# agiresearch/OpenP5

Measured on AMD Instinct MI355X. Metric: train_samples_per_sec, higher is better.
Workload: dtype bf16; 1 GPU; ML-1M-shaped sequential prompts, t5-small V=32100, B=64/GPU L=128 T=8, dropout 0.1, fwd+bwd+clip+AdamW (BASELINE.json configs[1]); global_batch=64, seq_len=128, tgt_len=8, parallelism=dp1

## Files before the change

### include/p5hip.h

```cpp
#ifndef P5HIP_H
#define P5HIP_H
#include <stddef.h>
#include <stdint.h>

#ifdef __cplusplus
extern "C" {
#endif

typedef struct P5Config {
  int vocab_size, d_model, d_kv, d_ff, n_enc_layers, n_dec_layers, n_heads;
  int rel_buckets, rel_max_distance, whole_word_size;
  int gated_gelu;
  int dtype;
  float eps, dropout;
  int pad_id, eos_id;
} P5Config;

typedef struct P5Engine P5Engine;

const char* p5_last_error(void);
int p5_set_option(const char* name, int value);
int p5_abi_version(void);
int p5_profile_begin(void);
int p5_profile_end(char* report, int cap);
// ... 233 lines not shown
                       const int* child_col, const uint32_t* excluded, int excl_words, float temperature, int rows, int T, int ldl, int ld_ref,
                       void* stream);
int p5_op_trie_reg_bwd(int dtype, void* dlogits, const float* logits, const float* ref_logits, const float* lse, const float* entropy, const float* kl,
                       const float* lse_ref, const int64_t* labels, const int* node, const int* state, const float* dnll, const float* d_entropy,
                       const float* d_kl, const int* child_off, const int* child_tok, const int* child_node, const int* child_col,
                       const uint32_t* excluded, int excl_words, float temperature, int rows, int T, int ldl, int ld_ref, int ldd,
                       const int64_t* out_attn, float gscale, float entropy_coef, float kl_coef, void* stream);
int p5_op_trunc_ce_fwd_cols(int dtype, float* nll, float* lse, float* row_cut, int* state, const float* logits, const int64_t* labels, const int* node,
                            const int* child_off, const int* child_tok, const int* child_node, const int* child_col, const uint32_t* excluded,
                            int excl_words, float temperature, int top_k, float top_p, int rows, int T, int ldl, void* stream);
int p5_op_trunc_ce_bwd_cols(int dtype, void* dlogits, const float* logits, const float* lse, const float* row_cut, const int64_t* labels, const int* node,
                            const int* state, const float* dnll, const int* child_off, const int* child_tok, const int* child_node, const int* child_col,
                            const uint32_t* excluded, int excl_words, float temperature, int rows, int T, int ldl, int ldd, const int64_t* out_attn,
                            float gscale, void* stream);
int p5_op_masked_mean(float* loss, const float* nll, const int64_t* out_attn, int B, int T, void* stream);
int p5_policy_batch(const int64_t* sequences, const int64_t* labels, const int64_t* output_attention, const float* rewards, int B, int S, int Ts,
                    int Tg, int baseline, float policy_coef, float sft_coef, int token_sum, float adv_eps, int with_gold, int pad_id, int eos_id,
                    int64_t* labels_out, int64_t* attention_out, float* rewards_out, float* advantages, float* weights_out, float* user_stats,
                    float* stats, void* stream);
int p5_op_skinny_gemm(int dtype, int amode, const void* A, int lda, const float* ln, const void* W, int ldw, void* C, int ldc,
                      int M, int N, int K, int epi, float alpha, float eps, void* stream);
int p5_op_dec_cross_attn(int dtype, int variant, void* out, const void* q, const void* kv, const int64_t* mask, int B, int H, int Kb,
                         int L, void* stream);
int p5_op_dec_cross_attn_ex(int dtype, int variant, void* out, const void* q, const float* x, const float* ln, const void* Wq, const void* kv,
                            int ldkv, const int64_t* mask, int B, int H, int Kb, int L, int d, float eps, const int* done, void* stream);
int p5_op_dec_self_attn(int dtype, void* out, const void* qkv, void* cache, const int* anc_odd, const int* anc_even, const float* rel_table,
                        const int* lut, int lut_half, int R, int H, const int* step, int max_len, const int* done, void* stream);
int p5_op_rmsnorm_f32in(int dtype, void* y, const float* x, const float* w, int rows, int d, float eps, const int* done, void* stream);
int p5_op_head_lse(int dtype, int nv, float* part_m, float* part_s, const void* hn, const void* E, int R, int d, int V, float alpha,
                   const int* done, void* stream);
// ... 41 lines not shown
```

### openp5_amd/_abi.py

```python
import ctypes as C

c_i64p = C.POINTER(C.c_int64)
vp, i32, i64, f32, f64, u32 = C.c_void_p, C.c_int, C.c_int64, C.c_float, C.c_double, C.c_uint32


class P5Config(C.Structure):
    _fields_ = [
        ("vocab_size", i32), ("d_model", i32), ("d_kv", i32), ("d_ff", i32), ("n_enc_layers", i32),
        ("n_dec_layers", i32), ("n_heads", i32), ("rel_buckets", i32), ("rel_max_distance", i32),
        ("whole_word_size", i32), ("gated_gelu", i32), ("dtype", i32), ("eps", f32), ("dropout", f32),
        ("pad_id", i32), ("eos_id", i32),
    ]


class P5GemmProblem(C.Structure):
    _fields_ = [("A", vp), ("B", vp), ("C", vp), ("aux", vp), ("M", i32), ("N", i32), ("K", i32), ("lda", i32), ("ldb", i32), ("ldc", i32),
                ("ldaux", i32), ("epi", i32), ("c_f32", i32), ("splitk", i32), ("alpha", f32), ("rowss", vp), ("rowss_eps", f32), ("ssq_out", vp), ("rowss_nt", i32), ("ssq_nt", i32),
                ("C2", vp), ("ldc2", i32), ("gate_F", i32),
                ("nb_dot", vp), ("nb_dot_nt", i32), ("nb_rin", vp), ("nb_rout", vp), ("nb_w", vp), ("nb_dw", vp)]


class P5EmbedBwdSet(C.Structure):
    _fields_ = [("key0", vp), ("key1", vp), ("dres0", vp), ("dres1", vp), ("n0", i32), ("n1", i32), ("site0", u32), ("site1", u32),
                ("drop_p0", f32), ("drop_p1", f32), ("table", vp), ("idx", vp), ("csort", vp), ("part", vp)]
# ... 101 lines not shown
    "p5_op_trie_ce_fwd": (i32, [i32, vp, vp, vp, vp, vp, vp, vp, vp, vp, vp, i32, f32, i32, i32, i32, vp]),
    "p5_op_trie_ce_bwd": (i32, [i32, vp, vp, vp, vp, vp, vp, vp, vp, vp, vp, vp, i32, f32, i32, i32, i32, i32, vp, f32, vp]),
    "p5_op_trunc_cut": (i32, [vp, vp, vp, vp, vp, vp, vp, vp, i32, f32, i32, f32, i32, i32, i32, vp]),
    "p5_op_trunc_ce_fwd": (i32, [i32, vp, vp, vp, vp, vp, vp, vp, vp, vp, vp, vp, i32, f32, i32, f32, i32, i32, i32, vp]),
    "p5_op_trunc_ce_bwd": (i32, [i32, vp, vp, vp, vp, vp, vp, vp, vp, vp, vp, vp, vp, i32, f32, i32, i32, i32, i32, vp, f32, vp]),
    "p5_op_item_gather": (i32, [i32, vp, vp, vp, i32, i32, vp]),
    "p5_op_item_scatter": (i32, [vp, vp, vp, i32, i32, i32, i32, vp]),
    "p5_op_trie_ce_fwd_cols": (i32, [i32, vp, vp, vp, vp, vp, vp, vp, vp, vp, vp, vp, i32, f32, i32, i32, i32, vp]),
    "p5_op_trie_ce_bwd_cols": (i32, [i32, vp, vp, vp, vp, vp, vp, vp, vp, vp, vp, vp, vp, i32, f32, i32, i32, i32, i32, vp, f32, vp]),
    "p5_op_trie_reg_fwd": (i32, [i32, vp, vp, vp, vp, vp, vp, vp, vp, vp, vp, vp, vp, vp, vp, vp, i32, f32, i32, i32, i32, i32, vp]),
    "p5_op_trie_reg_bwd": (i32, [i32, vp, vp, vp, vp, vp, vp, vp, vp, vp, vp, vp, vp, vp, vp, vp, vp, vp, vp, i32, f32, i32, i32, i32, i32, i32, vp, f32,
                                 f32, f32, vp]),
    "p5_op_trunc_ce_fwd_cols": (i32, [i32, vp, vp, vp, vp, vp, vp, vp, vp, vp, vp, vp, vp, i32, f32, i32, f32, i32, i32, i32, vp]),
    "p5_op_trunc_ce_bwd_cols": (i32, [i32, vp, vp, vp, vp, vp, vp, vp, vp, vp, vp, vp, vp, vp, i32, f32, i32, i32, i32, i32, vp, f32, vp]),
    "p5_op_masked_mean": (i32, [vp, vp, vp, i32, i32, vp]),
    "p5_policy_batch": (i32, [vp, vp, vp, vp, i32, i32, i32, i32, i32, f32, f32, i32, f32, i32, i32, i32, vp, vp, vp, vp, vp, vp, vp, vp]),
    "p5_op_dec_cross_attn": (i32, [i32, i32, vp, vp, vp, vp, i32, i32, i32, i32, vp]),
    "p5_op_skinny_gemm": (i32, [i32, i32, vp, i32, vp, vp, i32, vp, i32, i32, i32, i32, i32, f32, f32, vp]),
    "p5_op_dec_cross_attn_ex": (i32, [i32, i32, vp, vp, vp, vp, vp, vp, i32, vp, i32, i32, i32, i32, i32, f32, vp, vp]),
    "p5_op_dec_self_attn": (i32, [i32, vp, vp, vp, vp, vp, vp, vp, i32, i32, i32, vp, i32, vp, vp]),
    "p5_op_rmsnorm_f32in": (i32, [i32, vp, vp, vp, i32, i32, f32, vp, vp]),
    "p5_op_head_lse": (i32, [i32, i32, vp, vp, vp, vp, i32, i32, i32, f32, vp, vp]),
    "p5_op_dec_score": (i32, [i32, i32, vp, vp, i32, vp, vp, i32, f32, vp, i32, i32, vp, vp, vp, vp, vp, vp, i32, i32, i32, i32, i32, vp, vp, vp, vp, vp, vp]),
    "p5_op_head_nv": (i32, [i32, i32]),
    "p5_op_rank_select": (i32, [i32, vp, vp, i64, vp, i32, i32, vp, vp, i32, i32, vp, vp, vp, vp]),
    "p5_op_rank_edges": (i32, [i32, i32, vp, i64, vp, vp, i32, i32, vp, i32, vp, i32, i32, i32, i32, vp, vp, i32, vp, vp, vp]),
    "p5_op_cand_row_lse": (i32, [i32, i32, vp, vp, vp, i32, i32, vp, i32, i32, vp]),
    "p5_op_tree_attn": (i32, [i32, i32, vp, vp, vp, vp, i32, i32, i32, i32, i32, vp, vp, i32, vp, vp, i32, i32, vp]),
    "p5_op_cand_plan": (i32, [vp, vp, vp, vp, vp, vp, i32, i32, i32, i32, i32, i32, vp]),
    "p5_op_cand_rows": (i32, [vp, vp, i32, i32, i32, vp, vp, i32, i32, vp]),
# ... 30 lines not shown
```

### openp5_amd/csrc/p5_elem.h

```cpp
#pragma once
#include "p5_device.h"
#include "p5_rng.h"

template <class T>
__global__ __launch_bounds__(256) void p5_embed_fwd_kernel(T* __restrict__ out, const T* __restrict__ E, const T* __restrict__ WW,
                                                          const int64_t* __restrict__ ids, const int64_t* __restrict__ ww,
                                                          int rows, int d, P5Drop drop, float* __restrict__ ssq_part = nullptr) {
  constexpr int EPF = TT<T>::EPF;
  const int lane = threadIdx.x & 63;
  const int row = blockIdx.x * 4 + (threadIdx.x >> 6);
  if (row >= rows) return;
  const int64_t id = ids[row];
  const int64_t w = WW ? ww[row] : 0;
  const bool do_drop = drop.state != nullptr && drop.thr != 0;
  const uint32_t seed = p5_seed(drop);
  for (int c = lane; c < d / EPF; c += 64) {
    float x[8], y[8];
    unpack16<T>(ld16(E + (size_t)id * d + c * EPF), x);
    if (WW) {
      unpack16<T>(ld16(WW + (size_t)w * d + c * EPF), y);
#pragma unroll
      for (int e = 0; e < EPF; ++e) x[e] += y[e];
    }
    if (do_drop) {
#pragma unroll
      for (int e = 0; e < EPF; ++e)
        x[e] = p5_keep(seed, drop.site_key, (uint32_t)(row * d + c * EPF + e), drop.thr) ? x[e] * drop.scale : 0.f;
// ... 533 lines not shown
```

### openp5_amd/csrc/p5_embed.h

```cpp
#pragma once
#include "p5_device.h"
#include "p5_rng.h"

typedef int i32x4 __attribute__((ext_vector_type(4)));
#define P5_EMB_SEG 32
#define P5_EMB_MAXSETS 2

struct P5EmbSet {
  const int64_t* key0; const int64_t* key1;
  const float* dres0; const float* dres1;
  P5Drop drop0, drop1;
  float* table;
  int n0, n1;
  int* perm; int* sstart; int* slen;
  int* skey;
  unsigned long long* csort;
  float* part;
};
struct P5EmbArgs {
  P5EmbSet s[P5_EMB_MAXSETS];
  int nsets, d;
};

__device__ static __forceinline__ int emb_key(const P5EmbSet& s, int r) { return (int)(r < s.n0 ? s.key0[r] : s.key1[r - s.n0]); }
// ... 9 lines not shown
  __syncthreads();
  for (int k = 2; k <= P5_EMB_CHUNK; k <<= 1) {
    for (int j = k >> 1; j > 0; j >>= 1) {
      const int i = threadIdx.x, l = i ^ j;
      if (l > i) {
        const unsigned long long x = sv[i], y = sv[l];
        const bool up = (i & k) == 0;
        if ((x > y) == up) { sv[i] = y; sv[l] = x; }
      }
      __syncthreads();
    }
  }
  s.csort[(size_t)blockIdx.x * P5_EMB_CHUNK + threadIdx.x] = sv[threadIdx.x];
}

__device__ static __forceinline__ int emb_lower_bound(const unsigned long long* v, int m, unsigned long long x) {
  int lo = 0, hi = m;
#pragma unroll 1
  while (lo < hi) {
    const int mid = (lo + hi) >> 1;
    if (v[mid] < x) lo = mid + 1; else hi = mid;
  }
  return lo;
}

__global__ __launch_bounds__(256) void p5_embed_rank_kernel(P5EmbArgs a) {
  constexpr int CPB = 16;
  __shared__ unsigned long long sc[CPB * P5_EMB_CHUNK];
  __shared__ int scnt[3][4][64];
  const P5EmbSet& s = a.s[blockIdx.y];
  const int n = s.n0 + s.n1;
  if (blockIdx.x * 64 >= n) return;
  const int lane = threadIdx.x & 63, wave = threadIdx.x >> 6;
  const int r = blockIdx.x * 64 + lane;
  const int k = r < n ? emb_key(s, r) : 0;
  const unsigned long long me = (((unsigned long long)(unsigned)k) << 32) | (unsigned)r;
  const unsigned long long klo = ((unsigned long long)(unsigned)k) << 32, khi = ((unsigned long long)(unsigned)k + 1ull) << 32;
  const int nchunks = (n + P5_EMB_CHUNK - 1) / P5_EMB_CHUNK;
  int pos = 0, start = 0, end = 0;
  for (int c0 = 0; c0 < nchunks; c0 += CPB) {
    const int nc = nchunks - c0 < CPB ? nchunks - c0 : CPB;
    __syncthreads();
    for (int i = threadIdx.x; i < nc * P5_EMB_CHUNK; i += 256) sc[i] = s.csort[(size_t)c0 * P5_EMB_CHUNK + i];
    __syncthreads();
    for (int c = wave; c < nc; c += 4) {
      const unsigned long long* v = sc + c * P5_EMB_CHUNK;
      const int lo = emb_lower_bound(v, P5_EMB_CHUNK, klo);
      start += lo;
      const int hi = lo + emb_lower_bound(v + lo, P5_EMB_CHUNK - lo, khi);
      end += hi;
      pos += lo + emb_lower_bound(v + lo, hi - lo, me);
    }
  }
  scnt[0][wave][lane] = pos; scnt[1][wave][lane] = start; scnt[2][wave][lane] = end;
  __syncthreads();
  if (wave == 0 && r < n) {
    pos = scnt[0][0][lane] + scnt[0][1][lane] + scnt[0][2][lane] + scnt[0][3][lane];
    start = scnt[1][0][lane] + scnt[1][1][lane] + scnt[1][2][lane] + scnt[1][3][lane];
    end = scnt[2][0][lane] + scnt[2][1][lane] + scnt[2][2][lane] + scnt[2][3][lane];
    s.perm[pos] = r; s.skey[pos] = k; s.sstart[pos] = start; s.slen[pos] = end - start;
  }
}

__device__ static __forceinline__ void emb_row2(const P5EmbSet& s, int r, int d, int c, uint32_t seed0, uint32_t seed1, float& x0, float& x1) {
  const bool first = r < s.n0;
  const int lr = first ? r : r - s.n0;
  const float* src = (first ? s.dres0 : s.dres1) + (size_t)lr * d + c;
  const P5Drop& dp = first ? s.drop0 : s.drop1;
  x0 = src[0]; x1 = src[1];
  if (dp.state != nullptr && dp.thr != 0) {
    const uint32_t seed = first ? seed0 : seed1;
    const uint32_t i0 = (uint32_t)(lr * d + c);
    x0 = p5_keep(seed, dp.site_key, i0, dp.thr) ? x0 * dp.scale : 0.f;
    x1 = p5_keep(seed, dp.site_key, i0 + 1, dp.thr) ? x1 * dp.scale : 0.f;
  }
}

__global__ __launch_bounds__(256) void p5_embed_seg_kernel(P5EmbArgs a) {
  constexpr int S = P5_EMB_SEG;
  __shared__ int sp[S], sk[S], sst[S], sln[S];
  const P5EmbSet& s = a.s[blockIdx.y];
  const int n = s.n0 + s.n1, d = a.d;
  const int p0 = blockIdx.x * S;
  if (p0 >= n) return;
  const int cnt = n - p0 < S ? n - p0 : S;
  if (threadIdx.x < S) {
    const int p = p0 + threadIdx.x;
    const bool ok = threadIdx.x < cnt;
    sp[threadIdx.x] = ok ? s.perm[p] : 0; sk[threadIdx.x] = ok ? s.skey[p] : -1;
    sst[threadIdx.x] = ok ? s.sstart[p] : 0; sln[threadIdx.x] = ok ? s.slen[p] : 0;
  }
  __syncthreads();
  const uint32_t seed0 = p5_seed(s.drop0), seed1 = p5_seed(s.drop1);
  for (int c = threadIdx.x * 2; c < d; c += 512) {
    float v0[S], v1[S];
#pragma unroll
    for (int j = 0; j < S; ++j) {
      v0[j] = 0.f; v1[j] = 0.f;
      if (j < cnt) emb_row2(s, sp[j], d, c, seed0, seed1, v0[j], v1[j]);
    }
    float o0[S], o1[S];
#pragma unroll
    for (int j = 0; j < S; ++j) {
      o0[j] = 0.f; o1[j] = 0.f;
      if (j < cnt && (j == cnt - 1 || sk[j + 1] != sk[j])) {
        const int ss = sst[j], se = ss + sln[j];
        if (ss >= p0 && se <= p0 + S) {
          const float* src = s.table + (size_t)sk[j] * d + c;
          o0[j] = src[0]; o1[j] = src[1];
        }
      }
    }
    float a0 = 0.f, a1 = 0.f;
#pragma unroll
    for (int j = 0; j < S; ++j) {
      if (j >= cnt) break;
      a0 += v0[j]; a1 += v1[j];
      const bool last = j == cnt - 1 || sk[j + 1] != sk[j];
      if (last) {
        const int ss = sst[j], se = ss + sln[j];
        const bool head = ss < p0, tail = se > p0 + S;
        float* dst = (!head && !tail) ? s.table + (size_t)sk[j] * d + c : s.part + ((size_t)blockIdx.x * 2 + (head ? 0 : 1)) * d + c;
        if (!head && !tail) { dst[0] = o0[j] + a0; dst[1] = o1[j] + a1; } else { dst[0] = a0; dst[1] = a1; }
        a0 = 0.f; a1 = 0.f;
      }
    }
  }
}

__global__ __launch_bounds__(256) void p5_embed_fix_kernel(P5EmbArgs a) {
  constexpr int S = P5_EMB_SEG;
  const P5EmbSet& s = a.s[blockIdx.y];
  const int n = s.n0 + s.n1, d = a.d;
  const int p0 = blockIdx.x * S;
  if (p0 + S >= n) return;
  const int last = p0 + S - 1;
  const int ss = s.sstart[last], se = ss + s.slen[last];
  if (se <= p0 + S || ss < p0) return;
  const int key = s.skey[last];
  const int b1 = (se - 1) / S;
  for (int c = threadIdx.x * 2; c < d; c += 512) {
// ... 18 lines not shown
```

### openp5_amd/csrc/p5_lib.hip

```cpp
#include <string>
#include <vector>
#include <cstring>
#include <cstdio>
#include <cmath>
#include <cstdlib>
#ifndef P5_EMU
#include <dlfcn.h>
#endif

#include "p5_host.h"
#include "p5_elem.h"
#include "p5_embed.h"
#include "p5_decode.h"
#include "p5_decode2.h"
#include "p5_decode_wide.h"
#include "p5_verify.h"
#include "p5_rank.h"
#include "p5_cand.h"
#include "p5_prune.h"
#include "p5_bound.h"
#include "p5_sample.h"
#include "p5_sbs.h"
#include "p5_trie_ce.h"
#include "p5_trie_reg.h"
// ... 3 lines not shown
#include "../../include/p5hip.h"

thread_local std::string g_p5_err;

static int g_opt_wgrad_group = getenv("P5_WGRAD_GROUP") ? atoi(getenv("P5_WGRAD_GROUP")) : 1;
static int g_opt_dec_nb = getenv("P5_DEC_NB") ? atoi(getenv("P5_DEC_NB")) : 0;
static int g_opt_dec_kw = getenv("P5_DEC_KW") ? atoi(getenv("P5_DEC_KW")) : 0;
static int g_opt_dec_fuseq = getenv("P5_DEC_FUSEQ") ? atoi(getenv("P5_DEC_FUSEQ")) : 1;
static int g_opt_dgrad_t = getenv("P5_DGRAD_T") ? atoi(getenv("P5_DGRAD_T")) : 1;
static int g_opt_dec_cross = getenv("P5_DEC_CROSS") ? atoi(getenv("P5_DEC_CROSS")) : 3;
static int g_opt_dec_head = getenv("P5_DEC_HEAD") ? atoi(getenv("P5_DEC_HEAD")) : 1;
static int g_opt_dec_atomic = getenv("P5_DEC_ATOMIC") ? atoi(getenv("P5_DEC_ATOMIC")) : 0;
static int g_opt_adam_tiles = getenv("P5_ADAM_TILES") ? atoi(getenv("P5_ADAM_TILES")) : 1;
static int g_opt_gen_ff = getenv("P5_GEN_FF") ? atoi(getenv("P5_GEN_FF")) : 1;
static int g_opt_dec_head_nv = getenv("P5_DEC_HEAD_NV") ? atoi(getenv("P5_DEC_HEAD_NV")) : 0;
static int g_opt_gen_wide = getenv("P5_GEN_WIDE") ? atoi(getenv("P5_GEN_WIDE")) : 0;

__global__ __launch_bounds__(256) void p5_shift_right_kernel(int64_t* out, const int64_t* labels, int B, int T, int64_t start) {
  const int i = blockIdx.x * 256 + threadIdx.x;
  if (i >= B * T) return;
  const int t = i % T;
  int64_t v = (t == 0) ? start : labels[i - 1];
  if (v == -100) v = start;
  out[i] = v;
}

__global__ __launch_bounds__(64) void p5_tr_probe_kernel(unsigned short* out, const unsigned short* in) {
  __shared__ __attribute__((aligned(16))) unsigned short lds[256];
  const int l = threadIdx.x;
  for (int i = l; i < 256; i += 64) lds[i] = in[i];
  __syncthreads();
  const u32x2 r = lds_tr16_b64(&lds[(l >> 4) * 64 + (l & 15) * 4]);
  out[l * 4 + 0] = (unsigned short)(r[0] & 0xFFFF);
  out[l * 4 + 1] = (unsigned short)(r[0] >> 16);
  out[l * 4 + 2] = (unsigned short)(r[1] & 0xFFFF);
  out[l * 4 + 3] = (unsigned short)(r[1] >> 16);
}

static constexpr int P5_MAX_STAGED = 160;
// ... 54 lines not shown
  std::vector<LayerOff> enc, dec;
  std::vector<ParamInfo> table;
  float* P = nullptr; float* G = nullptr; void* S = nullptr;
  const int* lut_enc = nullptr; const int* lut_dec = nullptr; int lut_half = 0;
  uint32_t* rng = nullptr;
  int B = 0, L = 0, T = 0, training = 0, M = 0, Md = 0, Vp = 0;
  int Gt = 1, Bd = 0;
  const float* tgt_w = nullptr;
  const int64_t *ids = nullptr, *ww = nullptr, *mask = nullptr, *labels = nullptr, *out_attn = nullptr;
  std::vector<LayerSave> es, ds;
  void *enc_x0 = nullptr, *enc_xf = nullptr, *enc_out = nullptr; float* enc_rstd_f = nullptr;
  int64_t* dec_ids = nullptr; void *dec_x0 = nullptr, *dec_xf = nullptr, *dec_hn = nullptr; float* dec_rstd_f = nullptr;
  float *logits = nullptr, *lse_tok = nullptr, *ssq_scratch = nullptr;
  float *ce_part = nullptr, *ce_lab = nullptr, *ce_g = nullptr;
  bool ce_free_fwd = false;
  struct ItemLoss {
    bool on = false; P5TrieCe tr = {nullptr, nullptr, nullptr, nullptr, 0, 1.f}; int* state_out = nullptr;
    bool trunc = false; P5TruncCe tc = {0, 1.f}; float* row_cut = nullptr;
    bool head = false; const int* head_tok = nullptr; int Nu = 0, Nup = 0;
    void* head_ws = nullptr; size_t head_ws_bytes = 0;
    void *EU = nullptr, *dlogitsU = nullptr; float *logitsU = nullptr, *dEU = nullptr;
    bool reg = false; const float* ref = nullptr; int ld_ref = 0; float* row_terms = nullptr; float ent_coef = 0.f, kl_coef = 0.f;
    float* terms_out = nullptr;
  };
  ItemLoss il_next, il;
  const float *bw_dH = nullptr, *bw_dKL = nullptr;
  void* Sf = nullptr;
  float *dres_a = nullptr, *dres_b = nullptr, *d_enc = nullptr, *Dvec = nullptr, *dres_cur = nullptr, *rel_partial = nullptr;
  void *dy = nullptr, *dn = nullptr, *dqkv = nullptr, *dO = nullptr, *dh = nullptr, *du = nullptr, *dlogits = nullptr, *dkv = nullptr;
  void *dy2[P5_NSETS] = {}, *dh2[P5_NSETS] = {}, *du2[P5_NSETS] = {}, *dqkv2[P5_NSETS] = {}, *dkv2[P5_NSETS] = {};
// ... 781 lines not shown
  const int nd_ = c.n_dec_layers, ldkv = nd_ * 2 * in;
  {
    hipStream_t ks = e->side ? e->side : s;
    if (e->side) fork_to_side(e, s);
    P5_TRY(linear_fwd<T>(ks, e->enc_out, d, Wc<T>(e, e->dec[0].ca.k), e->ds[0].kv_ca, ldkv, M, 2 * in, d));
#ifndef P5_EMU
    if (e->side) hipEventRecord(e->kv_ev[0], e->side);
#endif
    if (nd_ > 1) {
      P5_TRY(linear_fwd<T>(ks, e->enc_out, d, Wc<T>(e, e->dec[1].ca.k), e->ds[1].kv_ca, ldkv, M, (nd_ - 1) * 2 * in, d));
#ifndef P5_EMU
      if (e->side) hipEventRecord(e->kv_ev[1], e->side);
#endif
    }
  }
  P5_LAUNCH(p5_shift_right_kernel, dim3((Md + 255) / 256), dim3(256), 0, s, e->dec_ids, e->labels, e->Bd, e->T, (int64_t)c.pad_id);
  P5_TRY(P5_KCHECK());
  const bool nf = norm_fused<T>(e);
  P5_LAUNCH((p5_embed_fwd_kernel<T>), dim3((Md + 3) / 4), dim3(256), 0, s, (T*)e->dec_x0, Wc<T>(e, e->off_E), (const T*)nullptr,
            (const int64_t*)e->dec_ids, (const int64_t*)nullptr, Md, d, mk_drop(e, 1, 0, 0), nf ? e->ds[0].ssq_sa : (float*)nullptr);
  P5_TRY(P5_KCHECK());
  for (int i = 0; i < c.n_dec_layers; ++i) {
    const LayerOff& lo = e->dec[i];
    LayerSave& l = e->ds[i];
    void* xnext = (i + 1 < c.n_dec_layers) ? e->ds[i + 1].x_sa : e->dec_xf;
    float* ssq_next = (i + 1 < c.n_dec_layers) ? e->ds[i + 1].ssq_sa : e->ssq_scratch;
    if (nf) {
      P5_TRY(gemm_nf<T>(s, l.x_sa, d, Wnf<T>(e, lo.sa.q), d, l.qkv, 3 * in, Md, 3 * in, d, P5_EPI_STORE, nullptr, 0, no_drop(), l.ssq_sa, c.eps, nullptr, d));
    } else {
      P5_TRY(rmsnorm_fwd<T>(s, l.n_sa, l.rstd_sa, l.x_sa, e->P + lo.sa.ln, Md, d, c.eps, no_drop()));
      P5_TRY(linear_fwd<T>(s, l.n_sa, d, Wc<T>(e, lo.sa.q), l.qkv, 3 * in, Md, 3 * in, d));
    }
    P5AttnArgs a;
    memset(&a, 0, sizeof(a));
    a.Q = l.qkv; a.K = (const T*)l.qkv + in; a.V = (const T*)l.qkv + 2 * in; a.O = l.o_sa; a.lse = l.lse_sa;
// ... 262 lines not shown
    if (e->tr_pending && e->tr_ev) { hipStreamWaitEvent(s, e->tr_ev, 0); hipStreamWaitEvent(e->side ? e->side : s, e->tr_ev, 0); }
#endif
    e->tr_pending = false;
#ifndef P5_EMU
    if (e->zg_pending && e->zg_ev) { hipStreamWaitEvent(s, e->zg_ev, 0); if (e->side) hipStreamWaitEvent(e->side, e->zg_ev, 0); }
#endif
    e->zg_pending = false;
    if (!dnll) P5_REQUIRE(e->out_attn, "backward without dnll needs p5_forward_loss (output_attention mask)");
    struct ItemGradsOnce { P5Engine* e; ~ItemGradsOnce() { e->bw_dH = e->bw_dKL = nullptr; } } item_grads_once{e};
    const float alpha = 1.0f / sqrtf((float)d);
    const bool hd = e->il.on && e->il.head;
    const float* hd_lg = hd ? (const float*)e->il.logitsU : (const float*)e->logits;
    void* hd_dl = hd ? e->il.dlogitsU : e->dlogits;
    const int hd_ld = hd ? e->il.Nup : e->Vp;
    if (e->ce_free_fwd) {
      P5_LAUNCH(p5_ce_gscale_kernel, dim3((Md + 255) / 256), dim3(256), 0, s, e->ce_g, e->labels, dnll, e->out_attn, e->T, 1.0f / (float)e->Bd, Md, e->tgt_w);
      P5_TRY(P5_KCHECK());
      P5GemmArgs g;
      memset(&g, 0, sizeof(g));
      g.A = e->dec_hn; g.B = Wc<T>(e, e->off_E); g.C = e->dlogits; g.M = Md; g.N = c.vocab_size; g.K = d; g.lda = d; g.ldb = d; g.ldc = e->Vp;
      g.epi = P5_EPI_CE_GRAD; g.alpha = alpha; g.drop = no_drop();
      g.ce_labels = e->labels; g.ce_lse = e->lse_tok; g.ce_g = e->ce_g; g.ce_np = (c.vocab_size + 63) / 64;
      P5_TRY(launch_gemm<T>(g, s));
    } else if (e->il.on && e->il.trunc) {
      P5_LAUNCH((p5_trunc_ce_bwd_kernel<T>), dim3(Md), dim3(256), 0, s, (T*)hd_dl, hd_lg, (const float*)e->lse_tok,
                (const float*)e->il.row_cut, e->labels, (const int*)e->ce_lab, (const int*)e->ce_g, dnll, e->il.tr, hd_ld, hd_ld, e->out_attn, e->T,
                1.0f / (float)e->Bd);
      P5_TRY(P5_KCHECK());
    } else if (e->il.on && e->il.reg) {
      const float* rt = e->il.row_terms;
      P5_LAUNCH((p5_trie_reg_bwd_kernel<T>), dim3(Md), dim3(256), 0, s, (T*)hd_dl, hd_lg, e->il.ref, (const float*)e->lse_tok, rt, rt + Md,
                rt + 2 * (size_t)Md, e->labels, (const int*)e->ce_lab, (const int*)e->ce_g, dnll, e->bw_dH, e->bw_dKL, e->il.tr, hd_ld, e->il.ld_ref,
// ... 1780 lines not shown
  else if (!strcmp(name, "gemm_ws")) g_opt_gemm_ws = value;
  else if (!strcmp(name, "gemm_ws128")) g_opt_gemm_ws128 = value;
  else if (!strcmp(name, "gemm_rect")) g_opt_gemm_rect = value;
  else if (!strcmp(name, "gemm_ws128_min_k")) g_opt_gemm_ws128_min_k = value;
  else if (!strcmp(name, "gate_fuse")) g_opt_gate_fuse = value;
  else if (!strcmp(name, "norm_bwd_blocks")) g_opt_norm_bwd_blocks = value;
  else if (!strcmp(name, "norm_bwd_fuse")) g_opt_norm_bwd_fuse = value;
  else if (!strcmp(name, "adam_tiles")) g_opt_adam_tiles = value;
  else if (!strcmp(name, "ce_free")) g_opt_ce_free = value;
  else if (!strcmp(name, "gemm_wide_min_tiles")) g_opt_gemm_wide_min_tiles = value;
  else if (!strcmp(name, "gemm_ring128_min_k")) g_opt_gemm_ring128_min_k = value;
  else if (!strcmp(name, "gemm_ring128_min_tiles")) g_opt_gemm_ring128_min_tiles = value;
  else if (!strcmp(name, "wgrad_wide_min")) g_opt_wgrad_wide_min = value;
  else if (!strcmp(name, "grad_store_first")) g_opt_grad_store_first = value;
  else if (!strcmp(name, "embed_det")) g_opt_embed_det = value;
  else if (!strcmp(name, "g4_nst")) g_opt_g4_nst = value;
  else if (!strcmp(name, "g4_wgs")) g_opt_g4_wgs = value;
  else return fail("p5_set_option: unknown option");
  return 0;
}
int p5_abi_version(void) { return 6; }
int p5_profile_begin(void) {
#ifndef P5_EMU
  P5Prof& p = p5_prof();
  p.recs.clear(); p.used = 0; p.pending_flops = 0.0; p.on = 1;
#else
  p5_emu_prof().recs.clear();
  p5_emu_prof().on = 1;
#endif
  return 0;
// ... 253 lines not shown
                       int B, int L, int T, int G, int training, float* nll_out, void* ws, int64_t ws_bytes, void* stream) {
  P5_REQUIRE(e->P, "engine not bound");
  P5_REQUIRE(B >= 1 && L >= 1 && L <= 512 && T >= 1 && T <= 512, "shape limits: 1 <= L,T <= 512");
  P5_REQUIRE(G >= 1, "targets per user: G >= 1");
  if (G > 1) {
    P5_REQUIRE((int64_t)G * T <= 512, "targets per user: G * T <= 512 (the cross-attention kernels' query limit)");
    P5_REQUIRE((int64_t)B * G * T <= P5_MAX_DEC_ROWS, "targets per user: B * G * T <= 65536 decoder rows");
    P5_REQUIRE((int64_t)B * G * e->c.n_heads <= 65535, "targets per user: B * G * n_heads <= 65535 (a launch grid's y extent)");
  }
  const int64_t need = layout_ws(e, (char*)ws, B, L, T, true, G);
  P5_REQUIRE(ws_bytes >= need, "workspace too small");
  P5_REQUIRE(((uintptr_t)ws % 256) == 0, "workspace must be 256-byte aligned");
  e->B = B; e->Gt = G; e->Bd = B * G; e->L = L; e->T = T; e->M = B * L; e->Md = B * G * T; e->training = training;
  e->Vp = (e->c.vocab_size + 63) / 64 * 64;
  e->ids = input_ids; e->ww = whole_word_ids; e->mask = attention_mask; e->labels = labels; e->out_attn = nullptr; e->tgt_w = nullptr;
  if (training && e->c.dropout > 0.f) P5_REQUIRE(e->rng, "training with dropout needs rng_state");
  e->il = e->il_next;
  e->il_next.on = false;
  e->il.tr.group = G;
  e->il.tr.tw = nullptr;
  if (e->il.on) P5_REQUIRE(nll_out, "item loss: nll_out");
  return e->c.dtype == 1 ? forward_impl<bf16>(e, nll_out, (hipStream_t)stream) : forward_impl<float>(e, nll_out, (hipStream_t)stream);
}
int p5_forward(P5Engine* e, const int64_t* input_ids, const int64_t* whole_word_ids, const int64_t* attention_mask, const int64_t* labels,
               int B, int L, int T, int training, float* nll_out, void* ws, int64_t ws_bytes, void* stream) {
  return p5_forward_targets(e, input_ids, whole_word_ids, attention_mask, labels, B, L, T, 1, training, nll_out, ws, ws_bytes, stream);
}
int p5_forward_loss_targets(P5Engine* e, const int64_t* input_ids, const int64_t* whole_word_ids, const int64_t* attention_mask, const int64_t* labels,
                            const int64_t* output_attention, int B, int L, int T, int G, const float* target_weights, int training, float* nll_out,
                            float* loss_out, void* ws, int64_t ws_bytes, void* stream) {
  P5_REQUIRE(output_attention && loss_out, "null argument");
  P5_TRY(p5_forward_targets(e, input_ids, whole_word_ids, attention_mask, labels, B, L, T, G, training, nll_out, ws, ws_bytes, stream));
  e->out_attn = output_attention;
  e->tgt_w = target_weights;
  e->il.tr.tw = target_weights;
  if (e->il.on && e->il.reg) {
    const float* rt = e->il.row_terms;
    P5_LAUNCH(p5_trie_reg_loss_kernel, dim3(1), dim3(256), 0, (hipStream_t)stream, loss_out, e->il.terms_out, (const float*)nll_out, rt,
              e->il.ref ? rt + e->Md : (const float*)nullptr, output_attention, B * G, T, target_weights, e->il.ent_coef, e->il.kl_coef);
    return P5_KCHECK();
  }
  P5_LAUNCH(p5_masked_mean_kernel, dim3(1), dim3(256), 0, (hipStream_t)stream, loss_out, (const float*)nll_out, output_attention, B * G, T, target_weights);
  return P5_KCHECK();
}
int p5_forward_loss(P5Engine* e, const int64_t* input_ids, const int64_t* whole_word_ids, const int64_t* attention_mask, const int64_t* labels,
                    const int64_t* output_attention, int B, int L, int T, int training, float* nll_out, float* loss_out, void* ws, int64_t ws_bytes,
                    void* stream) {
  return p5_forward_loss_targets(e, input_ids, whole_word_ids, attention_mask, labels, output_attention, B, L, T, 1, nullptr, training, nll_out, loss_out,
                                 ws, ws_bytes, stream);
}
int p5_train_set_item_loss(P5Engine* e, const int* child_off, const int* child_tok, const int* child_node, int n_nodes, const uint32_t* excluded_nodes,
                           int excluded_words, float temperature, int* row_state_out) {
  e->il_next.on = false;
  e->il_next.head = false;
  e->il_next.reg = false;
// ... 1070 lines not shown
                         top_k, top_p, rows, T, ldl, stream);
}
int p5_op_trunc_ce_bwd_cols(int dtype, void* dlogits, const float* logits, const float* lse, const float* row_cut, const int64_t* labels, const int* node,
                            const int* state, const float* dnll, const int* child_off, const int* child_tok, const int* child_node, const int* child_col,
                            const uint32_t* excluded, int excl_words, float temperature, int rows, int T, int ldl, int ldd, const int64_t* out_attn,
                            float gscale, void* stream) {
  P5_REQUIRE(child_col, "trunc_ce_bwd_cols: child_col");
  return op_trunc_ce_bwd(dtype, dlogits, logits, lse, row_cut, labels, node, state, dnll, child_off, child_tok, child_node, child_col, excluded, excl_words,
                         temperature, rows, T, ldl, ldd, out_attn, gscale, stream);
}
int p5_op_masked_mean(float* loss, const float* nll, const int64_t* out_attn, int B, int T, void* stream) {
  P5_REQUIRE(loss && nll && out_attn && B >= 1 && T >= 1, "masked_mean: arguments");
  P5_LAUNCH(p5_masked_mean_kernel, dim3(1), dim3(256), 0, (hipStream_t)stream, loss, nll, out_attn, B, T);
  return P5_KCHECK();
}
int p5_policy_batch(const int64_t* sequences, const int64_t* labels, const int64_t* output_attention, const float* rewards, int B, int S, int Ts, int Tg,
                    int baseline, float policy_coef, float sft_coef, int token_sum, float adv_eps, int with_gold, int pad_id, int eos_id,
                    int64_t* labels_out, int64_t* attention_out, float* rewards_out, float* advantages, float* weights_out, float* user_stats,
                    float* stats, void* stream) {
  P5_REQUIRE(sequences && labels && output_attention, "policy_batch: null input pointer (sequences, labels, output_attention)");
  P5_REQUIRE(labels_out && attention_out && rewards_out && advantages && weights_out && user_stats && stats, "policy_batch: null output pointer");
  P5_REQUIRE(B >= 1 && Ts >= 2 && Tg >= 1 && Tg <= (1 << 24), "policy_batch: shapes B >= 1, Ts >= 2, 1 <= Tg <= 2^24");
  P5_REQUIRE(S >= 1, "policy_batch: S >= 1 draws per user");
  P5_REQUIRE(S <= P5_POLICY_MAX_S, "policy_batch: S <= 1024 draws per user");
  P5_REQUIRE(baseline >= P5_BASELINE_NONE && baseline <= P5_BASELINE_GRPO, "policy_batch: unknown baseline (0 none, 1 mean, 2 loo, 3 grpo)");
  P5_REQUIRE(baseline != P5_BASELINE_LOO || S >= 2, "policy_batch: the loo baseline needs S >= 2");
  P5_REQUIRE(std::isfinite(policy_coef) && std::isfinite(sft_coef) && std::isfinite(adv_eps) && adv_eps >= 0.f, "policy_batch: non-finite coefficient (policy_coef, sft_coef, adv_eps)");
  P5_REQUIRE((token_sum == 0 || token_sum == 1) && (with_gold == 0 || with_gold == 1), "policy_batch: token_sum and with_gold are 0 or 1");
  P5PolicyArgs a;
  a.seq = sequences; a.labels = labels; a.out_attn = output_attention; a.rewards = rewards;
// ... 203 lines not shown
```

Before: 16040 samples/s.

## Fuse decoder shift into embed, merge loss mean with CE grad scale, rework embed-bwd kernels

```diff
diff --git a/include/p5hip.h b/include/p5hip.h
--- a/include/p5hip.h
+++ b/include/p5hip.h
@@ -271,6 +271,8 @@
                             const uint32_t* excluded, int excl_words, float temperature, int rows, int T, int ldl, int ldd, const int64_t* out_attn,
                             float gscale, void* stream);
 int p5_op_masked_mean(float* loss, const float* nll, const int64_t* out_attn, int B, int T, void* stream);
+int p5_op_masked_mean_g(int merged, float* loss, float* g_out, const float* nll, const int64_t* out_attn, const int64_t* labels, const float* tw, int B, int T,
+                        float gscale, void* stream);
 int p5_policy_batch(const int64_t* sequences, const int64_t* labels, const int64_t* output_attention, const float* rewards, int B, int S, int Ts,
                     int Tg, int baseline, float policy_coef, float sft_coef, int token_sum, float adv_eps, int with_gold, int pad_id, int eos_id,
                     int64_t* labels_out, int64_t* attention_out, float* rewards_out, float* advantages, float* weights_out, float* user_stats,
diff --git a/openp5_amd/_abi.py b/openp5_amd/_abi.py
--- a/openp5_amd/_abi.py
+++ b/openp5_amd/_abi.py
@@ -139,6 +139,7 @@
     "p5_op_trunc_ce_fwd_cols": (i32, [i32, vp, vp, vp, vp, vp, vp, vp, vp, vp, vp, vp, vp, i32, f32, i32, f32, i32, i32, i32, vp]),
     "p5_op_trunc_ce_bwd_cols": (i32, [i32, vp, vp, vp, vp, vp, vp, vp, vp, vp, vp, vp, vp, vp, i32, f32, i32, i32, i32, i32, vp, f32, vp]),
     "p5_op_masked_mean": (i32, [vp, vp, vp, i32, i32, vp]),
+    "p5_op_masked_mean_g": (i32, [i32, vp, vp, vp, vp, vp, vp, i32, i32, f32, vp]),
     "p5_policy_batch": (i32, [vp, vp, vp, vp, i32, i32, i32, i32, i32, f32, f32, i32, f32, i32, i32, i32, vp, vp, vp, vp, vp, vp, vp, vp]),
     "p5_op_dec_cross_attn": (i32, [i32, i32, vp, vp, vp, vp, i32, i32, i32, i32, vp]),
     "p5_op_skinny_gemm": (i32, [i32, i32, vp, i32, vp, vp, i32, vp, i32, i32, i32, i32, i32, f32, f32, vp]),
diff --git a/openp5_amd/csrc/p5_elem.h b/openp5_amd/csrc/p5_elem.h
--- a/openp5_amd/csrc/p5_elem.h
+++ b/openp5_amd/csrc/p5_elem.h
@@ -5,12 +5,21 @@
 template <class T>
 __global__ __launch_bounds__(256) void p5_embed_fwd_kernel(T* __restrict__ out, const T* __restrict__ E, const T* __restrict__ WW,
                                                           const int64_t* __restrict__ ids, const int64_t* __restrict__ ww,
-                                                          int rows, int d, P5Drop drop, float* __restrict__ ssq_part = nullptr) {
+                                                          int rows, int d, P5Drop drop, float* __restrict__ ssq_part = nullptr,
+                                                          const int64_t* __restrict__ shift_labels = nullptr, int64_t* __restrict__ ids_out = nullptr,
+                                                          int Tlen = 1, int64_t start = 0) {
   constexpr int EPF = TT<T>::EPF;
   const int lane = threadIdx.x & 63;
   const int row = blockIdx.x * 4 + (threadIdx.x >> 6);
   if (row >= rows) return;
-  const int64_t id = ids[row];
+  int64_t id;
+  if (shift_labels) {
+    id = row % Tlen == 0 ? start : shift_labels[row - 1];
+    if (id == -100) id = start;
+    if (lane == 0) ids_out[row] = id;
+  } else {
+    id = ids[row];
+  }
   const int64_t w = WW ? ww[row] : 0;
   const bool do_drop = drop.state != nullptr && drop.thr != 0;
   const uint32_t seed = p5_seed(drop);
diff --git a/openp5_amd/csrc/p5_embed.h b/openp5_amd/csrc/p5_embed.h
--- a/openp5_amd/csrc/p5_embed.h
+++ b/openp5_amd/csrc/p5_embed.h
@@ -47,19 +47,29 @@
   s.csort[(size_t)blockIdx.x * P5_EMB_CHUNK + threadIdx.x] = sv[threadIdx.x];
 }
 
-__device__ static __forceinline__ int emb_lower_bound(const unsigned long long* v, int m, unsigned long long x) {
-  int lo = 0, hi = m;
-#pragma unroll 1
-  while (lo < hi) {
-    const int mid = (lo + hi) >> 1;
-    if (v[mid] < x) lo = mid + 1; else hi = mid;
-  }
-  return lo;
-}
+__device__ static __forceinline__ void emb_count_below(const unsigned long long* const (&v)[2], const unsigned long long (&x)[3], int (&cnt)[2][3]) {
+  int p[2][3] = {};
+#pragma unroll
+  for (int s = P5_EMB_CHUNK / 2; s > 0; s >>= 1) {
+#pragma unroll
+    for (int h = 0; h < 2; ++h) {
+#pragma unroll
+      for (int q = 0; q < 3; ++q) p[h][q] += v[h][p[h][q] + s - 1] < x[q] ? s : 0;
+    }
+  }
+#pragma unroll
+  for (int h = 0; h < 2; ++h) {
+#pragma unroll
+    for (int q = 0; q < 3; ++q) cnt[h][q] = p[h][q] + (v[h][p[h][q]] < x[q] ? 1 : 0);
+  }
+}
+
+typedef unsigned long long emb_u64x2 __attribute__((ext_vector_type(2), aligned(8)));
 
 __global__ __launch_bounds__(256) void p5_embed_rank_kernel(P5EmbArgs a) {
   constexpr int CPB = 16;
-  __shared__ unsigned long long sc[CPB * P5_EMB_CHUNK];
+  constexpr int NLD = CPB * P5_EMB_CHUNK / 2 / 256;
+  __shared__ __attribute__((aligned(16))) unsigned long long sc[CPB * P5_EMB_CHUNK];
   __shared__ int scnt[3][4][64];
   const P5EmbSet& s = a.s[blockIdx.y];
   const int n = s.n0 + s.n1;
@@ -67,97 +77,142 @@
   const int lane = threadIdx.x & 63, wave = threadIdx.x >> 6;
   const int r = blockIdx.x * 64 + lane;
   const int k = r < n ? emb_key(s, r) : 0;
-  const unsigned long long me = (((unsigned long long)(unsigned)k) << 32) | (unsigned)r;
-  const unsigned long long klo = ((unsigned long long)(unsigned)k) << 32, khi = ((unsigned long long)(unsigned)k + 1ull) << 32;
+  const unsigned long long x[3] = {((unsigned long long)(unsigned)k) << 32, ((unsigned long long)(unsigned)k + 1ull) << 32,
+                                   (((unsigned long long)(unsigned)k) << 32) | (unsigned)r};
   const int nchunks = (n + P5_EMB_CHUNK - 1) / P5_EMB_CHUNK;
-  int pos = 0, start = 0, end = 0;
+  emb_u64x2 t[NLD];
+  auto fetch = [&](int c0) {
+    const int lim = (nchunks - c0 < CPB ? nchunks - c0 : CPB) * P5_EMB_CHUNK;
+    const unsigned long long* src = s.csort + (size_t)c0 * P5_EMB_CHUNK;
+#pragma unroll
+    for (int q = 0; q < NLD; ++q) {
+      const int i = (q * 256 + (int)threadIdx.x) * 2;
+      t[q] = *(const emb_u64x2*)(src + (i < lim ? i : 0));
+    }
+  };
+  fetch(0);
+  int tot[3] = {0, 0, 0};
   for (int c0 = 0; c0 < nchunks; c0 += CPB) {
     const int nc = nchunks - c0 < CPB ? nchunks - c0 : CPB;
     __syncthreads();
-    for (int i = threadIdx.x; i < nc * P5_EMB_CHUNK; i += 256) sc[i] = s.csort[(size_t)c0 * P5_EMB_CHUNK + i];
+#pragma unroll
+    for (int q = 0; q < NLD; ++q) *(emb_u64x2*)(sc + (q * 256 + (int)threadIdx.x) * 2) = t[q];
     __syncthreads();
-    for (int c = wave; c < nc; c += 4) {
-      const unsigned long long* v = sc + c * P5_EMB_CHUNK;
-      const int lo = emb_lower_bound(v, P5_EMB_CHUNK, klo);
-      start += lo;
-      const int hi = lo + emb_lower_bound(v + lo, P5_EMB_CHUNK - lo, khi);
-      end += hi;
-      pos += lo + emb_lower_bound(v + lo, hi - lo, me);
-    }
-  }
-  scnt[0][wave][lane] = pos; scnt[1][wave][lane] = start; scnt[2][wave][lane] = end;
+    if (c0 + CPB < nchunks) fetch(c0 + CPB);
+    for (int c = wave; c < nc; c += 8) {
+      const bool two = c + 4 < nc;
+      const unsigned long long* const v[2] = {sc + c * P5_EMB_CHUNK, sc + (two ? c + 4 : c) * P5_EMB_CHUNK};
+      int cnt[2][3];
+      emb_count_below(v, x, cnt);
+#pragma unroll
+      for (int q = 0; q < 3; ++q) tot[q] += cnt[0][q] + (two ? cnt[1][q] : 0);
+    }
+  }
+  scnt[0][wave][lane] = tot[2]; scnt[1][wave][lane] = tot[0]; scnt[2][wave][lane] = tot[1];
   __syncthreads();
   if (wave == 0 && r < n) {
-    pos = scnt[0][0][lane] + scnt[0][1][lane] + scnt[0][2][lane] + scnt[0][3][lane];
-    start = scnt[1][0][lane] + scnt[1][1][lane] + scnt[1][2][lane] + scnt[1][3][lane];
-    end = scnt[2][0][lane] + scnt[2][1][lane] + scnt[2][2][lane] + scnt[2][3][lane];
+    const int pos = scnt[0][0][lane] + scnt[0][1][lane] + scnt[0][2][lane] + scnt[0][3][lane];
+    const int start = scnt[1][0][lane] + scnt[1][1][lane] + scnt[1][2][lane] + scnt[1][3][lane];
+    const int end = scnt[2][0][lane] + scnt[2][1][lane] + scnt[2][2][lane] + scnt[2][3][lane];
     s.perm[pos] = r; s.skey[pos] = k; s.sstart[pos] = start; s.slen[pos] = end - start;
   }
 }
 
-__device__ static __forceinline__ void emb_row2(const P5EmbSet& s, int r, int d, int c, uint32_t seed0, uint32_t seed1, float& x0, float& x1) {
-  const bool first = r < s.n0;
-  const int lr = first ? r : r - s.n0;
-  const float* src = (first ? s.dres0 : s.dres1) + (size_t)lr * d + c;
-  const P5Drop& dp = first ? s.drop0 : s.drop1;
-  x0 = src[0]; x1 = src[1];
-  if (dp.state != nullptr && dp.thr != 0) {
-    const uint32_t seed = first ? seed0 : seed1;
-    const uint32_t i0 = (uint32_t)(lr * d + c);
-    x0 = p5_keep(seed, dp.site_key, i0, dp.thr) ? x0 * dp.scale : 0.f;
-    x1 = p5_keep(seed, dp.site_key, i0 + 1, dp.thr) ? x1 * dp.scale : 0.f;
+typedef float emb_f4 __attribute__((ext_vector_type(4), aligned(4)));
+#ifdef P5_EMU
+#define EMB_GLOBAL
+#else
+#define EMB_GLOBAL __attribute__((address_space(1)))
+#endif
+
+__device__ static __forceinline__ int emb_vzero() {
+  int z = 0;
+#ifndef P5_EMU
+  asm volatile("" : "+v"(z));
+#endif
+  return z;
+}
+
+template <int H0>
+__device__ static __forceinline__ void emb_seg_half(const P5EmbSet& s, const float* const* srow, const float* const* sown, const int* slr, const int* sk,
+                                                    const int* sst, const int* sln, int p0, int cnt, int d, int c, int z, uint32_t seed0, uint32_t seed1,
+                                                    bool use0, bool use1, float (&acc)[4]) {
+  constexpr int S = P5_EMB_SEG, HB = S / 2;
+  emb_f4 v[HB], o[HB];
+#pragma unroll
+  for (int i = 0; i < HB; ++i) v[i] = *(const EMB_GLOBAL emb_f4*)(srow[H0 + i + z] + c);
+#pragma unroll
+  for (int i = 0; i < HB; ++i) o[i] = *(const EMB_GLOBAL emb_f4*)(sown[H0 + i + z] + c);
+  P5_SCHED_FENCE();
+  if (use0 || use1) {
+#pragma unroll
+    for (int i = 0; i < HB; ++i) {
+      const int lr = slr[H0 + i];
+      const bool first = lr >= 0;
+      if (first ? use0 : use1) {
+        const uint32_t seed = first ? seed0 : seed1, site_key = first ? s.drop0.site_key : s.drop1.site_key;
+        const uint32_t thr = first ? s.drop0.thr : s.drop1.thr;
+        const float scale = first ? s.drop0.scale : s.drop1.scale;
+        const uint32_t i0 = (uint32_t)((lr & 0x7fffffff) * d + c);
+        v[i].x = p5_keep(seed, site_key, i0, thr) ? v[i].x * scale : 0.f;
+        v[i].y = p5_keep(seed, site_key, i0 + 1, thr) ? v[i].y * scale : 0.f;
+        v[i].z = p5_keep(seed, site_key, i0 + 2, thr) ? v[i].z * scale : 0.f;
+        v[i].w = p5_keep(seed, site_key, i0 + 3, thr) ? v[i].w * scale : 0.f;
+      }
+    }
+  }
+#pragma unroll
+  for (int i = 0; i < HB; ++i) {
+    const int j = H0 + i;
+    if (j < cnt) {
+      acc[0] += v[i].x; acc[1] += v[i].y; acc[2] += v[i].z; acc[3] += v[i].w;
+      if (sk[j + 1] != sk[j]) {
+        const int ss = sst[j], se = ss + sln[j];
+        const bool head = ss < p0, tail = se > p0 + S;
+        if (!head && !tail) {
+          *(emb_f4*)(s.table + (size_t)sk[j] * d + c) = (emb_f4){o[i].x + acc[0], o[i].y + acc[1], o[i].z + acc[2], o[i].w + acc[3]};
+        } else {
+          *(emb_f4*)(s.part + ((size_t)blockIdx.x * 2 + (head ? 0 : 1)) * d + c) = (emb_f4){acc[0], acc[1], acc[2], acc[3]};
+        }
+        acc[0] = 0.f; acc[1] = 0.f; acc[2] = 0.f; acc[3] = 0.f;
+      }
+    }
   }
 }
 
 __global__ __launch_bounds__(256) void p5_embed_seg_kernel(P5EmbArgs a) {
   constexpr int S = P5_EMB_SEG;
-  __shared__ int sp[S], sk[S], sst[S], sln[S];
+  __shared__ const float* srow[S];
+  __shared__ const float* sown[S];
+  __shared__ int slr[S], sk[S + 1], sst[S], sln[S];
   const P5EmbSet& s = a.s[blockIdx.y];
   const int n = s.n0 + s.n1, d = a.d;
   const int p0 = blockIdx.x * S;
   if (p0 >= n) return;
   const int cnt = n - p0 < S ? n - p0 : S;
   if (threadIdx.x < S) {
-    const int p = p0 + threadIdx.x;
-    const bool ok = threadIdx.x < cnt;
-    sp[threadIdx.x] = ok ? s.perm[p] : 0; sk[threadIdx.x] = ok ? s.skey[p] : -1;
-    sst[threadIdx.x] = ok ? s.sstart[p] : 0; sln[threadIdx.x] = ok ? s.slen[p] : 0;
+    const int t = threadIdx.x;
+    const bool ok = t < cnt;
+    const int p = p0 + (ok ? t : cnt - 1);
+    const int r = s.perm[p], key = s.skey[p], ss = s.sstart[p], ln = s.slen[p];
+    const int next = t + 1 < cnt ? s.skey[p + 1] : -1;
+    const bool first = r < s.n0;
+    const int lr = first ? r : r - s.n0;
+    const float* src = (first ? s.dres0 : s.dres1) + (size_t)lr * d;
+    const bool own = ok && next != key && ss >= p0 && ss + ln <= p0 + S;
+    srow[t] = src; sown[t] = own ? s.table + (size_t)key * d : src;
+    slr[t] = first ? lr : (lr | (int)0x80000000);
+    sk[t] = ok ? key : -1; sst[t] = ss; sln[t] = ln;
+    if (t == 0) sk[S] = -1;
   }
   __syncthreads();
   const uint32_t seed0 = p5_seed(s.drop0), seed1 = p5_seed(s.drop1);
-  for (int c = threadIdx.x * 2; c < d; c += 512) {
-    float v0[S], v1[S];
-#pragma unroll
-    for (int j = 0; j < S; ++j) {
-      v0[j] = 0.f; v1[j] = 0.f;
-      if (j < cnt) emb_row2(s, sp[j], d, c, seed0, seed1, v0[j], v1[j]);
-    }
-    float o0[S], o1[S];
-#pragma unroll
-    for (int j = 0; j < S; ++j) {
-      o0[j] = 0.f; o1[j] = 0.f;
-      if (j < cnt && (j == cnt - 1 || sk[j + 1] != sk[j])) {
-        const int ss = sst[j], se = ss + sln[j];
-        if (ss >= p0 && se <= p0 + S) {
-          const float* src = s.table + (size_t)sk[j] * d + c;
-          o0[j] = src[0]; o1[j] = src[1];
-        }
-      }
-    }
-    float a0 = 0.f, a1 = 0.f;
-#pragma unroll
-    for (int j = 0; j < S; ++j) {
-      if (j >= cnt) break;
-      a0 += v0[j]; a1 += v1[j];
-      const bool last = j == cnt - 1 || sk[j + 1] != sk[j];
-      if (last) {
-        const int ss = sst[j], se = ss + sln[j];
-        const bool head = ss < p0, tail = se > p0 + S;
-        float* dst = (!head && !tail) ? s.table + (size_t)sk[j] * d + c : s.part + ((size_t)blockIdx.x * 2 + (head ? 0 : 1)) * d + c;
-        if (!head && !tail) { dst[0] = o0[j] + a0; dst[1] = o1[j] + a1; } else { dst[0] = a0; dst[1] = a1; }
-        a0 = 0.f; a1 = 0.f;
-      }
-    }
+  const bool use0 = s.drop0.state != nullptr && s.drop0.thr != 0, use1 = s.drop1.state != nullptr && s.drop1.thr != 0;
+  const int z = emb_vzero();
+  for (int c = threadIdx.x * 4; c < d; c += 1024) {
+    float acc[4] = {0.f, 0.f, 0.f, 0.f};
+    emb_seg_half<0>(s, srow, sown, slr, sk, sst, sln, p0, cnt, d, c, z, seed0, seed1, use0, use1, acc);
+    if (cnt > S / 2) emb_seg_half<S / 2>(s, srow, sown, slr, sk, sst, sln, p0, cnt, d, c, z, seed0, seed1, use0, use1, acc);
   }
 }
 
diff --git a/openp5_amd/csrc/p5_lib.hip b/openp5_amd/csrc/p5_lib.hip
--- a/openp5_amd/csrc/p5_lib.hip
+++ b/openp5_amd/csrc/p5_lib.hip
@@ -41,6 +41,8 @@
 static int g_opt_adam_tiles = getenv("P5_ADAM_TILES") ? atoi(getenv("P5_ADAM_TILES")) : 1;
 static int g_opt_gen_ff = getenv("P5_GEN_FF") ? atoi(getenv("P5_GEN_FF")) : 1;
 static int g_opt_dec_head_nv = getenv("P5_DEC_HEAD_NV") ? atoi(getenv("P5_DEC_HEAD_NV")) : 0;
+static int g_opt_shift_fuse = getenv("P5_SHIFT_FUSE") ? atoi(getenv("P5_SHIFT_FUSE")) : 1;
+static int g_opt_loss_fuse = getenv("P5_LOSS_FUSE") ? atoi(getenv("P5_LOSS_FUSE")) : 1;
 static int g_opt_gen_wide = getenv("P5_GEN_WIDE") ? atoi(getenv("P5_GEN_WIDE")) : 0;
 
 __global__ __launch_bounds__(256) void p5_shift_right_kernel(int64_t* out, const int64_t* labels, int B, int T, int64_t start) {
@@ -50,6 +52,32 @@
   int64_t v = (t == 0) ? start : labels[i - 1];
   if (v == -100) v = start;
   out[i] = v;
+}
+
+__global__ __launch_bounds__(256) void p5_masked_mean_g_kernel(float* __restrict__ loss, float* __restrict__ g_out, const float* __restrict__ nll,
+                                                              const int64_t* __restrict__ out_attn, const int64_t* __restrict__ labels, int B, int T,
+                                                              float gscale, const float* __restrict__ tw = nullptr) {
+  __shared__ float sred[4];
+  float s = 0.f;
+  for (int b = threadIdx.x; b < B; b += 256) {
+    float num = 0.f, cnt = 0.f;
+    for (int t = 0; t < T; ++t) {
+      const float m = out_attn[(size_t)b * T + t] != 0 ? 1.f : 0.f;
+      num += nll[(size_t)b * T + t] * m;
+      cnt += m;
+    }
+    float r = num / fmaxf(cnt, 1.f);
+    if (tw) r *= tw[b];
+    s += r;
+    for (int t = 0; t < T; ++t) {
+      float g = out_attn[(size_t)b * T + t] != 0 ? gscale / fmaxf(cnt, 1.f) : 0.f;
+      if (tw) g *= tw[b];
+      if (labels[(size_t)b * T + t] == -100) g = 0.f;
+      g_out[(size_t)b * T + t] = g;
+    }
+  }
+  s = block_reduce(s, false, sred);
+  if (threadIdx.x == 0) loss[0] = s / (float)B;
 }
 
 __global__ __launch_bounds__(64) void p5_tr_probe_kernel(unsigned short* out, const unsigned short* in) {
@@ -134,6 +162,7 @@
   float *logits = nullptr, *lse_tok = nullptr, *ssq_scratch = nullptr;
   float *ce_part = nullptr, *ce_lab = nullptr, *ce_g = nullptr;
   bool ce_free_fwd = false;
+  bool ce_g_ready = false;
   struct ItemLoss {
     bool on = false; P5TrieCe tr = {nullptr, nullptr, nullptr, nullptr, 0, 1.f}; int* state_out = nullptr;
     bool trunc = false; P5TruncCe tc = {0, 1.f}; float* row_cut = nullptr;
@@ -945,11 +974,17 @@
 #endif
     }
   }
-  P5_LAUNCH(p5_shift_right_kernel, dim3((Md + 255) / 256), dim3(256), 0, s, e->dec_ids, e->labels, e->Bd, e->T, (int64_t)c.pad_id);
-  P5_TRY(P5_KCHECK());
   const bool nf = norm_fused<T>(e);
-  P5_LAUNCH((p5_embed_fwd_kernel<T>), dim3((Md + 3) / 4), dim3(256), 0, s, (T*)e->dec_x0, Wc<T>(e, e->off_E), (const T*)nullptr,
-            (const int64_t*)e->dec_ids, (const int64_t*)nullptr, Md, d, mk_drop(e, 1, 0, 0), nf ? e->ds[0].ssq_sa : (float*)nullptr);
+  if (g_opt_shift_fuse) {
+    P5_LAUNCH((p5_embed_fwd_kernel<T>), dim3((Md + 3) / 4), dim3(256), 0, s, (T*)e->dec_x0, Wc<T>(e, e->off_E), (const T*)nullptr,
+              (const int64_t*)nullptr, (const int64_t*)nullptr, Md, d, mk_drop(e, 1, 0, 0), nf ? e->ds[0].ssq_sa : (float*)nullptr, e->labels, e->dec_ids,
+              e->T, (int64_t)c.pad_id);
+  } else {
+    P5_LAUNCH(p5_shift_right_kernel, dim3((Md + 255) / 256), dim3(256), 0, s, e->dec_ids, e->labels, e->Bd, e->T, (int64_t)c.pad_id);
+    P5_TRY(P5_KCHECK());
+    P5_LAUNCH((p5_embed_fwd_kernel<T>), dim3((Md + 3) / 4), dim3(256), 0, s, (T*)e->dec_x0, Wc<T>(e, e->off_E), (const T*)nullptr,
+              (const int64_t*)e->dec_ids, (const int64_t*)nullptr, Md, d, mk_drop(e, 1, 0, 0), nf ? e->ds[0].ssq_sa : (float*)nullptr);
+  }
   P5_TRY(P5_KCHECK());
   for (int i = 0; i < c.n_dec_layers; ++i) {
     const LayerOff& lo = e->dec[i];
@@ -1242,8 +1277,11 @@
     void* hd_dl = hd ? e->il.dlogitsU : e->dlogits;
     const int hd_ld = hd ? e->il.Nup : e->Vp;
     if (e->ce_free_fwd) {
-      P5_LAUNCH(p5_ce_gscale_kernel, dim3((Md + 255) / 256), dim3(256), 0, s, e->ce_g, e->labels, dnll, e->out_attn, e->T, 1.0f / (float)e->Bd, Md, e->tgt_w);
-      P5_TRY(P5_KCHECK());
+      if (dnll || !e->ce_g_ready || !e->training) {
+        P5_LAUNCH(p5_ce_gscale_kernel, dim3((Md + 255) / 256), dim3(256), 0, s, e->ce_g, e->labels, dnll, e->out_attn, e->T, 1.0f / (float)e->Bd, Md, e->tgt_w);
+        P5_TRY(P5_KCHECK());
+        e->ce_g_ready = false;
+      }
       P5GemmArgs g;
       memset(&g, 0, sizeof(g));
       g.A = e->dec_hn; g.B = Wc<T>(e, e->off_E); g.C = e->dlogits; g.M = Md; g.N = c.vocab_size; g.K = d; g.lda = d; g.ldb = d; g.ldc = e->Vp;
@@ -3054,6 +3092,8 @@
   else if (!strcmp(name, "wgrad_wide_min")) g_opt_wgrad_wide_min = value;
   else if (!strcmp(name, "grad_store_first")) g_opt_grad_store_first = value;
   else if (!strcmp(name, "embed_det")) g_opt_embed_det = value;
+  else if (!strcmp(name, "shift_fuse")) g_opt_shift_fuse = value;
+  else if (!strcmp(name, "loss_fuse")) g_opt_loss_fuse = value;
   else if (!strcmp(name, "g4_nst")) g_opt_g4_nst = value;
   else if (!strcmp(name, "g4_wgs")) g_opt_g4_wgs = value;
   else return fail("p5_set_option: unknown option");
@@ -3337,6 +3377,7 @@
   e->B = B; e->Gt = G; e->Bd = B * G; e->L = L; e->T = T; e->M = B * L; e->Md = B * G * T; e->training = training;
   e->Vp = (e->c.vocab_size + 63) / 64 * 64;
   e->ids = input_ids; e->ww = whole_word_ids; e->mask = attention_mask; e->labels = labels; e->out_attn = nullptr; e->tgt_w = nullptr;
+  e->ce_g_ready = false;
   if (training && e->c.dropout > 0.f) P5_REQUIRE(e->rng, "training with dropout needs rng_state");
   e->il = e->il_next;
   e->il_next.on = false;
@@ -3362,6 +3403,13 @@
     P5_LAUNCH(p5_trie_reg_loss_kernel, dim3(1), dim3(256), 0, (hipStream_t)stream, loss_out, e->il.terms_out, (const float*)nll_out, rt,
               e->il.ref ? rt + e->Md : (const float*)nullptr, output_attention, B * G, T, target_weights, e->il.ent_coef, e->il.kl_coef);
     return P5_KCHECK();
+  }
+  if (g_opt_loss_fuse && training && e->ce_free_fwd && nll_out) {
+    P5_LAUNCH(p5_masked_mean_g_kernel, dim3(1), dim3(256), 0, (hipStream_t)stream, loss_out, e->ce_g, (const float*)nll_out, output_attention, e->labels, B * G, T,
+              1.0f / (float)e->Bd, target_weights);
+    P5_TRY(P5_KCHECK());
+    e->ce_g_ready = true;
+    return 0;
   }
   P5_LAUNCH(p5_masked_mean_kernel, dim3(1), dim3(256), 0, (hipStream_t)stream, loss_out, (const float*)nll_out, output_attention, B * G, T, target_weights);
   return P5_KCHECK();
@@ -4462,6 +4510,19 @@
   P5_LAUNCH(p5_masked_mean_kernel, dim3(1), dim3(256), 0, (hipStream_t)stream, loss, nll, out_attn, B, T);
   return P5_KCHECK();
 }
+int p5_op_masked_mean_g(int merged, float* loss, float* g_out, const float* nll, const int64_t* out_attn, const int64_t* labels, const float* tw, int B, int T,
+                        float gscale, void* stream) {
+  hipStream_t s = (hipStream_t)stream;
+  P5_REQUIRE(loss && g_out && nll && out_attn && labels && B >= 1 && T >= 1, "masked_mean_g: arguments");
+  if (merged) {
+    P5_LAUNCH(p5_masked_mean_g_kernel, dim3(1), dim3(256), 0, s, loss, g_out, nll, out_attn, labels, B, T, gscale, tw);
+    return P5_KCHECK();
+  }
+  P5_LAUNCH(p5_masked_mean_kernel, dim3(1), dim3(256), 0, s, loss, nll, out_attn, B, T, tw);
+  P5_TRY(P5_KCHECK());
+  P5_LAUNCH(p5_ce_gscale_kernel, dim3((B * T + 255) / 256), dim3(256), 0, s, g_out, labels, (const float*)nullptr, out_attn, T, gscale, B * T, tw);
+  return P5_KCHECK();
+}
 int p5_policy_batch(const int64_t* sequences, const int64_t* labels, const int64_t* output_attention, const float* rewards, int B, int S, int Ts, int Tg,
                     int baseline, float policy_coef, float sft_coef, int token_sum, float adv_eps, int with_gold, int pad_id, int eos_id,
                     int64_t* labels_out, int64_t* attention_out, float* rewards_out, float* advantages, float* weights_out, float* user_stats,
```

Result: faster. 16200 samples/s (median of 6 runs) (+1.0%).
